# jhamrick/gaussian_processes

Hardware: AMD Instinct MI355X
Metric: GP fit+predict wall-clock (kernel build + Cholesky + solve + log_lh + posterior mean) (lower is better)
Workload: dtype f64; 1 GPU; N=65536 d=32 RBF(GaussianKernel) f64, m=1000 test points, h=1 w=0.5*sqrt(d) s=1; N=65536, d=32, m=1000, parallelism=1 GPU

## Files before the change

### gaussian_processes_amd/csrc/gpx_common.h

```cpp
#pragma once
#include <hip/hip_runtime.h>
#include <stdint.h>
#include <stdio.h>
#include <stdlib.h>
#include <string.h>
#include <math.h>
#include <vector>

#include "../../include/gpx.h"
#include "gpx_tune.h"

namespace gpx {

void set_error(const char *fmt, ...);
int  hip_fail(hipError_t e, const char *what, const char *file, int line);
int  ensure_device();

#define GPX_HIP(call)                                                        \
    do {                                                                     \
        hipError_t e__ = (call);                                             \
        if (e__ != hipSuccess) return gpx::hip_fail(e__, #call, __FILE__, __LINE__); \
    } while (0)

#define GPX_TRY(call)                                                        \
// ... 95 lines not shown

struct KParams {
    double c[6];
    double diag_add;
    int kernel;
    int member;
};
int make_kparams(int kernel, int member, const double *params, double diag_add, KParams *out);

struct Batch {
    int count; int64_t sA, sB, sC;
    int count2 = 1; int64_t tA = 0, tB = 0, tC = 0;
};

int gemm_nt(int dtype, int64_t M, int64_t N, int64_t K, const void *A, int64_t lda, const void *B,
            int64_t ldb, void *C, int64_t ldc, double alpha, int tri, int64_t row0, int64_t col0,
            hipStream_t st, int beta0 = 0, int ktri = 0, const Batch *bt = nullptr,
            int wide_tiles = 0);
int trsm_rows(int dtype, void *X, int64_t ldx, int64_t rows, const void *Ljj, int64_t ldl, int jb,
              hipStream_t st, const Batch *bt = nullptr);
int syrk_bc(int dtype, int64_t n, int64_t row_begin, void *Cloc, int64_t ldc, int64_t cl0, int64_t cl1,
            const void *Pb, int64_t ldp, int64_t k0, int64_t kb, int64_t nb, int P, int rank,
            hipStream_t st, const int *abort_flag = nullptr, const Batch *bt = nullptr);
struct PanelHints { bool idle_chip = false; int leaf_force = 0; };
struct PotrfHook { int (*fn)(void *user, int64_t cols_done, hipEvent_t panel_done); void *user; };
int potrf_panel(int dtype, void *A, int64_t lda, int64_t n, int64_t r0, int64_t c0, int64_t kb,
                int *info_dev, hipStream_t st, const Batch *bt = nullptr, int64_t kpre = 0,
                hipEvent_t done = nullptr, PanelHints hints = {});
int potrf(int dtype, void *A, int64_t n, int64_t lda, int *info_dev, hipStream_t st, const Batch *bt = nullptr,
          int64_t xrows = 0,
          bool may_block = false,
          const PotrfHook *hook = nullptr);
int potrf_panel_res(int dtype, void *A, int64_t lda, int64_t n, int64_t r0, int64_t c0, int64_t kb, int *info_dev,
                    hipStream_t st, const Batch *bt = nullptr, int64_t kpre = 0, hipEvent_t done = nullptr, PanelHints hints = {});
int64_t panel_res_max();
hipStream_t potrf_side_stream();
bool kernel_values_finite(int kernel, const double *p, double s, int dtype);
bool panel_res_fold(int64_t rows, int64_t kpre, int64_t kb, size_t es, int64_t lda, const void *base);
constexpr int TRSV_OPS_BLOCK = 512;
static inline int64_t trsv_ops_nblocks(int64_t n) { return n / TRSV_OPS_BLOCK; }
static inline bool trsv_ops_whole_blocks(int64_t n) { return n >= TRSV_OPS_BLOCK && n % TRSV_OPS_BLOCK == 0; }
struct TrsvOps {
    GrowBuf mem;
    bool valid = false;
    int64_t built = 0;
    void invalidate() { valid = false; built = 0; }
    static TrsvOps view(void *p, size_t bytes) { TrsvOps o; o.mem.p = p; o.mem.bytes = bytes; return o; }
};
int trsv_ops_build(int dtype, const void *L, int64_t n, int64_t ldl, TrsvOps *ops, hipStream_t st);
bool trsv_ops_ahead_ok(int dtype, const void *L, int64_t n, int64_t ldl);
bool trsm_ops_ok(int dtype, const void *L, int64_t n, int64_t ldl);
size_t trsv_ops_bytes(int dtype, int64_t n);
int trsv_ops_build_upto(int dtype, const void *L, int64_t n, int64_t ldl, TrsvOps *ops, int64_t kend, hipStream_t st);
int trsv_lower(int dtype, const void *L, int64_t n, int64_t ldl, void *b, void *x, int transpose,
               hipStream_t st, const Batch *bt = nullptr,
               TrsvOps *ops = nullptr);
int trsm_right_lt(int dtype, const void *L, int64_t n, int64_t ldl, void *X, int64_t m, int64_t ldx,
                  hipStream_t st, int x_upper = 0, TrsvOps *ops = nullptr,
                  int64_t c0 = 0);
int trsm_right_l(int dtype, const void *L, int64_t n, int64_t ldl, void *X, int64_t m, int64_t ldx, hipStream_t st,
                 TrsvOps *ops = nullptr);
int pred_grad(int dtype, int kernel, const void *xo, int64_t m, const void *x, int64_t n, int d, const double *params,
              const void *alpha, const void *B, int64_t ldb, double scale, const double *col_div, double *out_dev, hipStream_t st);
int inv_from_factor(int dtype, const void *L, int64_t n, int64_t ldl, void *X, void *W, int tri, hipStream_t st,
                    TrsvOps *ops, int count = 1, int64_t sL = 0, void *group_ops = nullptr);
int logdet_chol(int dtype, const void *L, int64_t n, int64_t ldl, double *out_dev, hipStream_t st, int count = 1,
                int64_t sL = 0, int64_t so = 0);
int dot(int dtype, const void *a, const void *b, int64_t n, double *out_dev, hipStream_t st, int count = 1,
        int64_t sa = 0, int64_t sb = 0, int64_t so = 0);
int tril(int dtype, void *A, int64_t n, int64_t lda, hipStream_t st);
int var_rows(int dtype, int kernel, const void *X, int64_t rows, int64_t n, int64_t ldx, const void *xo, int d,
             const double *params, const double *kdiag_dev, int accumulate, double *out_dev, hipStream_t st);
int var_finish(int dtype, int kernel, const void *xo, int d, const double *params, const double *acc_dev, int64_t rows,
               double *out_dev, hipStream_t st);
int eye_rows(int dtype, void *X, int64_t rows, int64_t ld, int64_t c0, int64_t cz, hipStream_t st);
int loo_rows(int dtype, const void *X, int64_t rows, int64_t n, int64_t ldx, int64_t c0, const void *y, const void *alpha,
             double *kii, double *mean, double *var, double *logp, hipStream_t st);
int loo_points(int dtype, const double *kii, const void *y, const void *alpha, int64_t n, double *mean, double *var, double *logp,
               hipStream_t st);
int sum_f64(const double *a, int64_t n, double *out_dev, hipStream_t st);
int copy_lower(int dtype, const void *src, int64_t lds, void *dst, int64_t ldd, int64_t n, hipStream_t st);
int schur_lower(int dtype, const void *B, int64_t k, int64_t n, int64_t ldb, void *S, int64_t lds, hipStream_t st);
int randn(int dtype, void *out, int64_t rows, int64_t cols, int64_t ld, uint64_t seed, uint64_t stream, uint64_t offset, hipStream_t st);
int mvn_sample(int dtype, void *C, int64_t m, int64_t ldc, const void *mean, double jitter, int64_t S, uint64_t seed, uint64_t stream,
               void *Z, int64_t ldz, void *out, int64_t ldo, int *info_dev, hipStream_t st);
bool kapply_fused_fits(int dtype, int d, int64_t S);
int kapply_fused(int dtype, const void *xo, int64_t m, const void *x, int64_t n, int d, const KParams &kp, const void *V, int64_t ldv,
                 int64_t S, void *out, int64_t ldo, hipStream_t st);
int rff_features(int dtype, const void *pts, int64_t m, int d, const double *omega_dev, int64_t F, double scale, void *out, int64_t ld,
                 hipStream_t st);
int rff_features_grad(int dtype, const void *pts, int64_t m, int d, const double *omega_dev, int64_t F, double scale, const double *col_div,
                      void *out, int64_t ld, hipStream_t st);
int kapply_grad(int dtype, const void *xo, int64_t m, const void *x, int64_t n, int d, const double *params, const double *col_div,
                const void *V, int64_t ldv, int64_t S, void *out, int64_t ldo, hipStream_t st);
int kmat_apply(int dtype, int kernel, const void *xo, int64_t m, const void *x, int64_t n, int d, const double *params, const void *V,
               int64_t ldv, int64_t S, void *out, int64_t ldo, hipStream_t st);
int var_plan(int dtype, int64_t n, int64_t m, int64_t chunk_rows, size_t free_bytes, int64_t *rows, int64_t *chunks, size_t *bytes);
int dloglh_reduce(int dtype, int kernel, const void *x, int64_t n, int d, const double *params,
                  const void *alpha, const void *W, int64_t ldw, double *partial_dev, double *out4,
                  hipStream_t st);
struct ArdWidths { double w[GPX_ARD_MAX_D]; };
int scale_points(int dtype, const void *x, int64_t n, int d, const double *w_host, void *out, hipStream_t st);
int ard_scratch(size_t bytes, void **p);
void ard_iso(const double *params, int d, double *iso2);
size_t dloglh_partial_doubles(int kernel, int d);
int dloglh_reduce_ard(int dtype, const void *xs, int64_t n, int d, const double *iso, const void *alpha, const void *W,
// ... 6 lines not shown
```

### gaussian_processes_amd/csrc/gpx_gp.hip

```cpp
#include "gpx_common.h"
#include <cmath>
#include <vector>

#include "gpx_gp_internal.h"

namespace gpx {

template <typename T>
__global__ void cvt_from_f64_2d(const double *__restrict__ src, int64_t lds, T *__restrict__ dst, int64_t ldd, int64_t rows, int64_t cols)
{
    const int64_t c = (int64_t)blockIdx.x * blockDim.x + threadIdx.x;
    if (c >= cols) return;
    for (int64_t r = blockIdx.y; r < rows; r += gridDim.y) dst[r * ldd + c] = (T)src[r * lds + c];
}

template <typename T>
__global__ void cvt_to_f64_2d(const T *__restrict__ src, int64_t lds, double *__restrict__ dst,
                              int64_t ldd, int64_t rows, int64_t cols, int lower_only)
{
    const int64_t c = (int64_t)blockIdx.x * blockDim.x + threadIdx.x;
    if (c >= cols) return;
    for (int64_t r = blockIdx.y; r < rows; r += gridDim.y) {
        const double v = (double)src[r * lds + c];
        dst[r * ldd + c] = (lower_only && c > r) ? 0.0 : v;
// ... 38 lines not shown
                           cols, rows, cols, lower_only);
    else
        hipLaunchKernelGGL((cvt_to_f64_2d<float>), grid, block, 0, st, (const float *)src, lds, tmp, cols,
                           rows, cols, lower_only);
    GPX_LAUNCH_CHECK();
    GPX_TRY(copy_rows(dst, ldh, tmp, cols, rows, cols, hipMemcpyDeviceToHost, st));
    GPX_HIP(hipStreamSynchronize(st));
    return GPX_OK;
}

int kmat(int dtype, int kernel, int member, const void *x1, int64_t n, const void *x2, int64_t m,
         int d, const double *params, double diag_add, int tri, void *out, int64_t ld, hipStream_t st)
{
    return gpx_d_kmat(dtype, kernel, member, x1, n, x2, m, d, params, diag_add, tri, out, ld, (void *)st);
}

int gp_rescale(gpx_gp *g)
{
    if (g->kernel != GPX_KERNEL_GAUSSIAN_ARD || !g->have_data || !g->have_params) return GPX_OK;
    ard_iso(g->params, g->d, g->iso);
    return scale_points(g->dtype, g->x, g->n, g->d, g->params + 1, g->xs, g->st);
}

static int upload_points(gpx_gp *g, void *dst, const double *xo, int64_t m)
{
    GPX_TRY(upload_f64(g->dtype, dst, m * g->d, xo, m * g->d, 1, m * g->d, g->st));
    if (g->kernel == GPX_KERNEL_GAUSSIAN_ARD) GPX_TRY(scale_points(g->dtype, dst, m, g->d, g->params + 1, dst, g->st));
    return GPX_OK;
}

int gp_read_scal(gpx_gp *g, GpScal *host)
{
    GPX_HIP(hipMemcpyAsync(host, g->scal, sizeof(GpScal), hipMemcpyDeviceToHost, g->st));
    GPX_HIP(hipStreamSynchronize(g->st));
    return check_internal_info(host->info);
}

int gp_need_factor(gpx_gp *g, const char *what_for)
{
    GpScal sc;
    GPX_TRY(gp_read_scal(g, &sc));
    if (sc.info != 0) { set_error("Kxx is not positive definite (info = %d): there is no factor %s", sc.info, what_for); return GPX_ERR_ARG; }
    return GPX_OK;
}

int check_internal_info(int info)
{
    if (info >= 0) return GPX_OK;
    set_error("internal failure inside the factorisation (info = %d: a hand-off between workgroups of the resident "
              "panel kernel timed out); the factor is not valid -- this is NOT a statement about the matrix", info);
    return GPX_ERR_INTERNAL;
}

int gp_finish_fit(gpx_gp *g, bool rhs_is_row_n, int *info)
{
    const size_t es = esize(g->dtype);
    hipStream_t st = g->st;
    if (rhs_is_row_n) {
        GPX_TRY(trsv_lower(g->dtype, g->A, g->n, g->lda, (char *)g->A + (size_t)g->n * g->lda * es, g->alpha, 1, st, nullptr, &g->ops));
    } else {
        GPX_HIP(hipMemcpyAsync(g->t0, g->y, (size_t)g->n * es, hipMemcpyDeviceToDevice, st));
        GPX_TRY(trsv_lower(g->dtype, g->A, g->n, g->lda, g->t0, g->t1, 0, st, nullptr, &g->ops));
        GPX_TRY(trsv_lower(g->dtype, g->A, g->n, g->lda, g->t1, g->alpha, 1, st, nullptr, &g->ops));
    }
    GPX_HIP(hipEventRecord(g->ev[3], st));
    GPX_TRY(logdet_chol(g->dtype, g->A, g->n, g->lda, &g->scal->logdet, st));
    GPX_TRY(dot(g->dtype, g->y, g->alpha, g->n, &g->scal->yta, st));
    GPX_HIP(hipEventRecord(g->ev[4], st));
    g->fitted = true;
    if (info) {
        GPX_HIP(hipMemcpyAsync(info, &g->scal->info, sizeof(int), hipMemcpyDeviceToHost, st));
        GPX_HIP(hipStreamSynchronize(st));
        GPX_TRY(check_internal_info(*info));
    }
    return GPX_OK;
}

template <typename T>
__global__ void nonfinite_kernel(const T *__restrict__ v, int64_t n, int *__restrict__ flag)
{
    bool bad = false;
    for (int64_t i = (int64_t)blockIdx.x * blockDim.x + threadIdx.x; i < n; i += (int64_t)gridDim.x * blockDim.x)
        bad = bad || !isfinite(v[i]);
    if (__any(bad) && (threadIdx.x & 63) == 0) atomicOr(flag, 1);
}

int gp_scan_finite(gpx_gp *g)
{
    int *flags = &g->scal->x_bad;
    GPX_HIP(hipMemsetAsync(flags, 0, 2 * sizeof(int), g->st));
    const int64_t nx = g->n * g->d, ny = g->n;
    const unsigned bx = (unsigned)std::min<int64_t>(cdiv(nx, 256), 1024), by = (unsigned)std::min<int64_t>(cdiv(ny, 256), 1024);
    if (g->dtype == GPX_F64) {
        hipLaunchKernelGGL((nonfinite_kernel<double>), dim3(bx), dim3(256), 0, g->st, (const double *)g->x, nx, flags);
        hipLaunchKernelGGL((nonfinite_kernel<double>), dim3(by), dim3(256), 0, g->st, (const double *)g->y, ny, flags + 1);
    } else {
        hipLaunchKernelGGL((nonfinite_kernel<float>), dim3(bx), dim3(256), 0, g->st, (const float *)g->x, nx, flags);
        hipLaunchKernelGGL((nonfinite_kernel<float>), dim3(by), dim3(256), 0, g->st, (const float *)g->y, ny, flags + 1);
    }
    GPX_LAUNCH_CHECK();
    int h[2] = {0, 0};
    GPX_HIP(hipMemcpyAsync(h, flags, sizeof(h), hipMemcpyDeviceToHost, g->st));
    GPX_HIP(hipStreamSynchronize(g->st));
    g->x_finite = h[0] == 0; g->y_finite = h[1] == 0;
    return GPX_OK;
}

template <typename T>
static bool kernel_values_finite_t(int kernel, const double *p, double s)
{
    T k0, k1;
    if (kernel == GPX_KERNEL_GAUSSIAN) {
// ... 169 lines not shown
{
    GP_ENTER(g);
    GPX_ARG(g && x && y, "NULL argument");
    GPX_TRY(upload_f64(g->dtype, g->x, g->n * g->d, x, g->n * g->d, 1, g->n * g->d, g->st));
    GPX_TRY(upload_f64(g->dtype, g->y, g->n, y, g->n, 1, g->n, g->st));
    g->have_data = true; gp_unfit(g);
    GPX_TRY(gp_rescale(g));
    return gp_scan_finite(g);
}

int gpx_gp_set_data_device(gpx_gp_t *g, const void *x_dev, const void *y_dev)
{
    GP_ENTER(g);
    GPX_ARG(g && x_dev && y_dev, "NULL argument");
    const size_t es = esize(g->dtype);
    GPX_HIP(hipMemcpyAsync(g->x, x_dev, (size_t)g->n * g->d * es, hipMemcpyDeviceToDevice, g->st));
    GPX_HIP(hipMemcpyAsync(g->y, y_dev, (size_t)g->n * es, hipMemcpyDeviceToDevice, g->st));
    GPX_HIP(hipStreamSynchronize(g->st));
    g->have_data = true; gp_unfit(g);
    GPX_TRY(gp_rescale(g));
    return gp_scan_finite(g);
}

int gpx_gp_set_params(gpx_gp_t *g, const double *params, double s)
{
    GP_ENTER(g);
    GPX_ARG(g && params, "NULL argument");
    GPX_ARG(!(s < 0), "invalid value for s");
    for (int i = 0; i < g->nparams; ++i) g->params[i] = params[i];
    g->s = s;
    g->have_params = true; g->have_K = false; gp_unfit(g);
    return gp_rescale(g);
}

int gpx_gp_get_params(gpx_gp_t *g, double *params, int cap, int *count)
{
    GP_ENTER(g);
    GPX_ARG(g->have_params, "no kernel parameters in the handle");
    GPX_ARG(cap >= 0 && (cap == 0 || params), "bad arguments");
    if (count) *count = g->nparams;
    for (int i = 0; i < g->nparams && i < cap; ++i) params[i] = g->params[i];
    return GPX_OK;
}

int gpx_gp_set_K(gpx_gp_t *g, const double *Kxx, int64_t ld)
{
    GP_ENTER(g);
    GPX_ARG(g && Kxx && ld >= g->n, "bad arguments");
    GPX_TRY(upload_f64(g->dtype, g->A, g->lda, Kxx, ld, g->n, g->n, g->st));
    g->have_K = true; gp_unfit(g);
    return GPX_OK;
}

struct OpsAhead { gpx_gp *g; int64_t group, last; };
static int ops_ahead_step(void *user, int64_t cols_done, hipEvent_t panel_done)
{
    OpsAhead *o = (OpsAhead *)user;
    gpx_gp *g = o->g;
    const int64_t ready = std::min(trsv_ops_nblocks(cols_done), o->last);
    if (ready - g->ops.built < o->group) return GPX_OK;
    GPX_HIP(hipStreamWaitEvent(g->st_ops, panel_done, 0));
    return trsv_ops_build_upto(g->dtype, g->A, g->n, g->lda, &g->ops, ready, g->st_ops);
}

int gpx_gp_fit(gpx_gp_t *g, int *info)
{
    GP_ENTER(g);
    GPX_ARG(g, "gp is NULL");
    GPX_ARG(g->have_data && (g->have_params || g->have_K),
            "set_data and set_params (or set_K) must be called before fit");
    const GpView v = gp_view(g);
    if (!g->have_K && (!g->x_finite || !kernel_values_finite(v.kernel, v.params, g->s, g->dtype))) {
        set_error("%s (%s)", NONFINITE_MSG, g->x_finite ? "kernel parameters or s" : "x");
        return GPX_ERR_ARG;
    }
    const size_t es = esize(g->dtype);
    hipStream_t st = g->st;
    GPX_HIP(hipEventRecord(g->ev[0], st));
    if (!g->have_K)
        GPX_TRY(kmat(g->dtype, v.kernel, GPX_K, v.x, g->n, v.x, g->n, g->d, v.params, g->s * g->s,
                     GPX_LOWER, g->A, g->lda, st));
    g->have_K = false;
    g->have_kii = false;
    GPX_HIP(hipEventRecord(g->ev[1], st));
    const int64_t ride_max = tune().fit_ride_max;
    const bool ride = g->n <= ride_max;
    route_hit(ride ? RT_FIT_RIDE : RT_FIT_TWO_SOLVES);
    if (ride) GPX_HIP(hipMemcpyAsync((char *)g->A + (size_t)g->n * g->lda * es, g->y, (size_t)g->n * es, hipMemcpyDeviceToDevice, st));
    g->ops.invalidate();
    const bool ahead = tune().fit_ops_ahead != 0 && g->n >= tune().fit_ops_ahead_min &&
                       trsv_ops_ahead_ok(g->dtype, g->A, g->n, g->lda);
    const int64_t nfull = trsv_ops_nblocks(g->n), tail = tune().fit_ops_tail;
    const int64_t group = std::max<int64_t>(1, std::min(nfull, nfull - tail));
    OpsAhead oa = {g, group, std::max<int64_t>(0, nfull - tail)};
    PotrfHook hook = {ops_ahead_step, &oa};
    if (ahead) {
        if (!g->st_ops) {
            int least = 0, greatest = 0;
            GPX_HIP(hipDeviceGetStreamPriorityRange(&least, &greatest));
            GPX_HIP(hipStreamCreateWithPriority(&g->st_ops, hipStreamNonBlocking, least));
            GPX_HIP(hipEventCreateWithFlags(&g->ev_ops, hipEventDisableTiming));
        }
        GPX_TRY(g->ops.mem.reserve(trsv_ops_bytes(g->dtype, g->n), st));
        GPX_TRY(order(g->ev_ops, st, g->st_ops));
    }
    GPX_TRY(potrf(g->dtype, g->A, g->n, g->lda, &g->scal->info, st, nullptr, ride ? 1 : 0, true, ahead ? &hook : nullptr));
    if (ahead) {
        GPX_TRY(order(g->ev_ops, g->st_ops, st));
        if (g->ops.built > 0) route_hit(RT_FIT_OPS_AHEAD);
    }
    GPX_HIP(hipEventRecord(g->ev[2], st));
    return gp_finish_fit(g, ride, info);
}

static int gp_scalars(gpx_gp_t *g, double *logdet, double *yta, int *info)
{
    GP_ENTER(g);
    GPX_ARG(g && g->fitted, "gp is not fitted");
    GpScal sc;
    GPX_TRY(gp_read_scal(g, &sc));
    if (logdet) *logdet = sc.logdet;
    if (yta) *yta = sc.yta;
    if (info) *info = sc.info;
    return GPX_OK;
}

int gpx_gp_log_lh(gpx_gp_t *g, double *log_lh)
{
    GPX_ARG(log_lh, "log_lh is NULL");
    GPX_ARG(g, "gp is NULL");
    GP_NEED_FINITE_Y(g);
    double logdet, yta; int info;
    GPX_TRY(gp_scalars(g, &logdet, &yta, &info));
    if (info != 0 || !(logdet >= GPX_MIN_LOG)) { *log_lh = -INFINITY; return GPX_OK; }
    const double data_fit = -0.5 * yta;
    const double complexity_penalty = -0.5 * logdet;
    const double constant = -0.5 * (double)g->n * log(2 * M_PI);
    *log_lh = data_fit + complexity_penalty + constant;
    return GPX_OK;
}

int gpx_gp_logdet(gpx_gp_t *g, double *logdet)
{
    GPX_ARG(logdet, "logdet is NULL");
    return gp_scalars(g, logdet, nullptr, nullptr);
}

int gpx_gp_info(gpx_gp_t *g, int *info)
{
    GPX_ARG(info, "info is NULL");
    return gp_scalars(g, nullptr, nullptr, info);
}

int gpx_gp_mean(gpx_gp_t *g, const double *xo, int64_t m, double *out)
{
    GP_ENTER(g);
    GPX_ARG(g && g->fitted, "gp is not fitted");
    GP_NEED_FINITE_Y(g);
    GPX_ARG(m >= 0 && (m == 0 || (xo && out)), "bad arguments");
    if (m == 0) return GPX_OK;
    const size_t es = esize(g->dtype);
    DevBuf dxo, dout;
    GPX_TRY(dxo.alloc((size_t)m * g->d * es));
    GPX_TRY(dout.alloc((size_t)m * es));
    GPX_TRY(upload_points(g, dxo.p, xo, m));
// ... 690 lines not shown
```

### gaussian_processes_amd/csrc/gpx_gp_internal.h

```cpp
#pragma once
#include "gpx_common.h"
#include <cstddef>

struct GpScal {
    double logdet;
    double yta;
    int x_bad, y_bad;
    int info;
    int pad;
};
static_assert(sizeof(GpScal) == 32 && offsetof(GpScal, x_bad) == 16 && offsetof(GpScal, info) == 24, "GpScal layout");

struct gpx_gp {
    int device;
    int dtype, kernel, d, nparams;
    int64_t n, lda;
    void *x, *y, *A, *alpha, *t0, *t1;
    void *xs;
    GpScal *scal;
    hipStream_t st;
    hipEvent_t ev[6];
    double params[1 + GPX_ARD_MAX_D];
    double iso[2];
    double s;
    bool have_data, have_params, fitted, have_K;
    bool x_finite, y_finite;
    gpx::GrowBuf bw; int64_t bw_cap;
    gpx::TrsvOps ops;
    gpx::GrowBuf gw; int64_t gw_cap;
    gpx::TrsvOps bops;
    double *kii;
    bool have_kii;
    hipStream_t st_ops;
    hipEvent_t ev_ops;
};

namespace gpx {
int gp_scan_finite(gpx_gp *g);
int upload_f64(int dtype, void *dst, int64_t ldd, const double *src, int64_t lds, int64_t rows, int64_t cols, hipStream_t st,
               DevBuf *stage = nullptr);
int download_f64(int dtype, double *dst, int64_t ldh, const void *src, int64_t lds, int64_t rows, int64_t cols, int lower_only,
                 hipStream_t st);
int gp_read_scal(gpx_gp *g, GpScal *host);
int gp_need_factor(gpx_gp *g, const char *what_for);
static inline void gp_unfit(gpx_gp *g) { g->fitted = false; g->have_kii = false; }
int gp_finish_fit(gpx_gp *g, bool rhs_is_row_n, int *info);
static inline int nparams_of(int kernel, int d) { return kernel == GPX_KERNEL_GAUSSIAN_ARD ? 1 + d : (kernel == GPX_KERNEL_PERIODIC ? 3 : 2); }
struct GpView { int kernel; const void *x; const double *params; };
static inline GpView gp_view(const gpx_gp *g)
{
    if (g->kernel == GPX_KERNEL_GAUSSIAN_ARD) return {GPX_KERNEL_GAUSSIAN, g->xs, g->iso};
    return {g->kernel, g->x, g->params};
}
int gp_rescale(gpx_gp *g);
}

#define GP_ENTER(g)                                                          \
    GPX_ARG((g) != nullptr, "gp is NULL");                                   \
    gpx::tune_refresh();                                                     \
    gpx::DeviceGuard guard__((g)->device);                                   \
    if (guard__.rc != GPX_OK) return guard__.rc;                             \
    gpx::StreamTurn turn__((g)->st);                                         \
    gpx::RoctxRange api_range__(__func__)
```

### gaussian_processes_amd/csrc/gpx_potrf.hip

```cpp
#include "gpx_common.h"
#include "gpx_leaf.h"
#include <vector>

namespace gpx {

constexpr int IBP = IB + 1;


template <typename T, bool INV>
__global__ __launch_bounds__(256) void potrf_diag_kernel(T *__restrict__ blk, int64_t lda, int64_t j0,
                                                         int jb, int *__restrict__ info, T *__restrict__ inv,
                                                         int64_t sblk)
{
    blk += (int64_t)blockIdx.x * sblk;
    info += blockIdx.x;
    if (INV) inv += (int64_t)blockIdx.x * (IB * IB);
    __builtin_amdgcn_s_setprio(3);
    const int tid = threadIdx.x;
    const int tr = tid >> 4, tc = tid & 15;
    __shared__ int s_abort;
    if (tid == 0) s_abort = *info;
    __syncthreads();
    if (s_abort != 0) return;
    T a[4][4];
// ... 98 lines not shown
}

template <typename T>
__global__ void tril_kernel(T *__restrict__ A, int64_t n, int64_t lda)
{
    for (int64_t i = blockIdx.y; i < n; i += gridDim.y)
        for (int64_t c = i + 1 + (int64_t)blockIdx.x * blockDim.x + threadIdx.x; c < n;
             c += (int64_t)gridDim.x * blockDim.x)
            A[i * lda + c] = (T)0;
}

int tril(int dtype, void *A, int64_t n, int64_t lda, hipStream_t st)
{
    if (n <= 1) return GPX_OK;
    dim3 grid((unsigned)std::min<int64_t>(cdiv(n, 256), 64), (unsigned)std::min<int64_t>(n, 32768)), block(256);
    if (dtype == GPX_F64) hipLaunchKernelGGL((tril_kernel<double>), grid, block, 0, st, (double *)A, n, lda);
    else hipLaunchKernelGGL((tril_kernel<float>), grid, block, 0, st, (float *)A, n, lda);
    GPX_LAUNCH_CHECK();
    return GPX_OK;
}

static int64_t outer_block(int64_t n, bool batched = false)
{
    const int64_t forced = tune().potrf_nb;
    if (forced >= IB && forced % IB == 0) return forced;
    if (batched && n >= 8192 && n <= 32768) return 1024;
    if (batched && n >= 4096 && n <= 32768) return 512;
    const long long *thr = tune().potrf_widths;
    if (n <= thr[0]) return 128;
    if (n <= thr[1]) return 256;
    if (n <= thr[2]) return 512;
    return 1024;
}

static thread_local ThreadScratch g_leaf;

template <typename T>
static int potrf_panel_t(T *A, int64_t lda, int64_t n, int64_t r0, int64_t c0, int64_t kb, int *info_dev,
                         hipStream_t st, int dtype, const Batch *bt, int64_t kpre = 0, hipEvent_t done = nullptr,
                         PanelHints hints = {})
{
    const int nbatch = bt ? bt->count : 1;
    const int64_t sM = bt ? bt->sA : 0;
    if (kb % IB == 0 && kb <= panel_res_max()) {
        route_hit(RT_PANEL_RES);
        return potrf_panel_res(dtype, A, lda, n, r0, c0, kb, info_dev, st, bt, kpre, done, hints);
    }
    if (kpre != 0) { set_error("potrf_panel: a folded update needs the resident panel route"); return GPX_ERR_ARG; }
    if (kb <= IB) {
        route_hit(RT_PANEL_CHAIN);
        const int jb = (int)kb;
        T *D = A + r0 * lda + c0;
        const int64_t below = n - (r0 + jb);
        const bool via_inverse = !tune().potrf_trsm_rows && below > 0 && below <= tune().potrf_inv_max &&
                                 jb == IB && lda % (16 / (int64_t)sizeof(T)) == 0 &&
                                 ((uintptr_t)(A + (r0 + jb) * lda + c0)) % 16 == 0;
        T *inv = nullptr;
        if (via_inverse) {
            void *p = nullptr;
            GPX_TRY(g_leaf.get(std::max<size_t>((size_t)nbatch * IB * IB * sizeof(T), IB * IB * 8), &p));
            inv = (T *)p;
        }
        {
            ProfScope prof(PC_POTRF_DIAG, (double)jb * jb * jb / 3.0 * nbatch, st);
            if (inv)
                hipLaunchKernelGGL((potrf_diag_kernel<T, true>), dim3(nbatch), dim3(256), 0, st, D, lda, r0, jb,
                                   info_dev, inv, sM);
            else
                hipLaunchKernelGGL((potrf_diag_kernel<T, false>), dim3(nbatch), dim3(256), 0, st, D, lda, r0, jb,
                                   info_dev, inv, sM);
        }
        GPX_LAUNCH_CHECK();
        if (via_inverse) {
            T *Xb = A + (r0 + jb) * lda + c0;
            Batch bi; bi.count = nbatch; bi.sA = sM; bi.sB = IB * IB; bi.sC = sM;
            GPX_TRY(gemm_nt(dtype, below, jb, jb, Xb, lda, inv, IB, Xb, lda, 1.0, GPX_FULL, 0, 0, st, 1, 0,
                            bt ? &bi : nullptr));
        } else if (below > 0) {
            Batch br; br.count = nbatch; br.sA = sM; br.sB = sM; br.sC = 0;
            GPX_TRY(trsm_rows(dtype, A + (r0 + jb) * lda + c0, lda, below, D, lda, jb, st, bt ? &br : nullptr));
        }
        if (done) GPX_HIP(hipEventRecord(done, st));
        return GPX_OK;
    }
    const int64_t h = ((kb / IB + 1) / 2) * IB;
    GPX_TRY(potrf_panel_t<T>(A, lda, n, r0, c0, h, info_dev, st, dtype, bt, 0, nullptr, hints));
    hints.idle_chip = false;
    T *R = A + (r0 + h) * lda + c0;
    if (panel_res_fold(n - (r0 + h), h, kb - h, sizeof(T), lda, A))
        return potrf_panel_t<T>(A, lda, n, r0 + h, c0 + h, kb - h, info_dev, st, dtype, bt, h, done, hints);
    GPX_TRY(gemm_nt(dtype, n - (r0 + h), kb - h, h, R, lda, R, lda, R + h, lda, -1.0, GPX_LOWER, 0, 0, st, 0, 0, bt));
    return potrf_panel_t<T>(A, lda, n, r0 + h, c0 + h, kb - h, info_dev, st, dtype, bt, 0, done, hints);
}

int potrf_panel(int dtype, void *A, int64_t lda, int64_t n, int64_t r0, int64_t c0, int64_t kb,
                int *info_dev, hipStream_t st, const Batch *bt, int64_t kpre, hipEvent_t done, PanelHints hints)
{
    if (dtype == GPX_F64)
        return potrf_panel_t<double>((double *)A, lda, n, r0, c0, kb, info_dev, st, dtype, bt, kpre, done, hints);
    return potrf_panel_t<float>((float *)A, lda, n, r0, c0, kb, info_dev, st, dtype, bt, kpre, done, hints);
}

struct LookAhead { hipStream_t q = nullptr; EventPool ev; };
static thread_local PerDevice<LookAhead> g_la;

hipStream_t potrf_side_stream()
{
// ... 198 lines not shown
```

### gaussian_processes_amd/csrc/gpx_solve.hip

```cpp
#include "gpx_common.h"
#include "gpx_kernels_dev.h"
#include "gpx_leaf.h"

namespace gpx {

constexpr int SB = 64;
constexpr int OB = TRSV_OPS_BLOCK;

template <typename T>
__global__ __launch_bounds__(256) void inv64_kernel(const T *__restrict__ L, int64_t ldl, int64_t ncols,
                                                    T *__restrict__ out, int transposed, T *__restrict__ W,
                                                    T *__restrict__ Wt, int64_t bsL, int64_t bsOut)
{
    L += (int64_t)blockIdx.y * bsL;
    const int tid = threadIdx.x, tr = tid >> 4, tc = tid & 15;
    const int64_t k0 = (int64_t)blockIdx.x * SB;
    const int jb = (int)min((int64_t)SB, ncols - k0);
    const T *blk = L + k0 * ldl + k0;
    T a[4][4], x[4][4];
#pragma unroll
    for (int r = 0; r < 4; ++r)
#pragma unroll
        for (int c = 0; c < 4; ++c) {
            const int row = 4 * tr + r, col = 4 * tc + c;
// ... 492 lines not shown
struct Sweep {
    const T *L; int64_t n, ldl, ncols; T *b, *x; hipStream_t st;
    unsigned nbt; int64_t sL, sv;
    T *Linv; int64_t sLinv;
    int aligned;
    int64_t nb() const { return cdiv(ncols, TB); }
    int width(int64_t blk) const { return (int)std::min<int64_t>(TB, ncols - blk * TB); }
};

template <typename T>
static void inv64_blocks(const Sweep<T> &S, int64_t first, int transposed)
{
    hipLaunchKernelGGL((inv64_kernel<T>), dim3((unsigned)(cdiv(S.ncols, SB) - first), S.nbt), dim3(256), 0, S.st,
                       S.L + first * SB * (S.ldl + 1), S.ldl, S.ncols - first * SB, S.Linv + first * SB * SB, transposed,
                       (T *)nullptr, (T *)nullptr, S.sL, S.sLinv);
}

template <typename T>
static void steps_fwd(const Sweep<T> &S, int64_t kfirst)
{
    const int64_t n = S.n, nb = S.nb();
    auto launch = [&](int64_t far_rows, int64_t nn, int64_t k0, int jb, int64_t p0, int pjb, int64_t far0) {
        hipLaunchKernelGGL((trsv_fwd_fused<T>), dim3((unsigned)(1 + cdiv(far_rows, 64)), S.nbt), dim3(TBT), 0, S.st, S.L, S.ldl,
                           S.Linv, S.b, S.x, nn, k0, jb, p0, pjb, far0, S.aligned, S.sL, S.sLinv, S.sv);
    };
    for (int64_t blk = kfirst; blk < nb; ++blk) {
        const int64_t k0 = blk * TB, p0 = std::max<int64_t>(blk - 1, 0) * TB;
        const int jb = S.width(blk), pjb = blk > 0 ? TB : 0;
        if (blk > 0) launch(jb, k0 + jb, k0, 0, p0, pjb, k0);
        launch(blk > 0 ? n - (k0 + jb) : 0, n, k0, jb, p0, pjb, k0 + jb);
    }
    if (n > S.ncols) launch(n - S.ncols, n, S.ncols, 0, (nb - 1) * TB, S.width(nb - 1), S.ncols);
}

template <typename T>
static void steps_bwd(const Sweep<T> &S, int64_t kfirst)
{
    const int64_t nb = S.nb();
    for (int64_t blk = nb - 1; blk >= kfirst; --blk) {
        const int64_t k0 = blk * TB, q0 = k0 + TB;
        const int jb = S.width(blk), qjb = blk + 1 < nb ? S.width(blk + 1) : 0;
        if (qjb > 0)
            hipLaunchKernelGGL((trsv_bwd_fused<T, 32>), dim3((unsigned)(1 + cdiv(jb, 32)), S.nbt), dim3(TBT), 0, S.st, S.L,
                               S.ldl, S.Linv, S.b, S.x, k0, 0, q0, qjb, k0, k0 + jb, S.aligned, S.sL, S.sLinv, S.sv);
        hipLaunchKernelGGL((trsv_bwd_fused<T, 128>), dim3((unsigned)(1 + (qjb > 0 ? cdiv(k0, 128) : 0)), S.nbt),
                           dim3(TBT), 0, S.st, S.L, S.ldl, S.Linv, S.b, S.x, k0, jb, q0, qjb, (int64_t)0, k0, S.aligned,
                           S.sL, S.sLinv, S.sv);
    }
}

constexpr int NCH = OB / (TBT / OPL);

template <typename T>
static void ops_fwd(const Sweep<T> &S, const OpsView<T> &V)
{
    for (int64_t k = 0; k < V.nfull; ++k) {
        const int64_t k0 = k * OB, far0 = k0 + OB;
        const int64_t nfar = k > 0 ? cdiv(S.n - far0, 64) : 0;
        hipLaunchKernelGGL((trsv_op_kernel<T, true>), dim3((unsigned)(NCH + nfar)), dim3(TBT), 0, S.st, V.W(k),
                           k > 0 ? V.Tf(k) : (const T *)nullptr, S.L, S.ldl, S.b, S.x, S.n, k0, k0 - OB, k > 0 ? OB : 0, far0, S.n, NCH, 1);
    }
}

template <typename T>
static void ops_bwd(const Sweep<T> &S, const OpsView<T> &V, int64_t kend)
{
    for (int64_t k = kend - 1; k >= 0; --k) {
        const int64_t k0 = k * OB, q0 = k0 + OB;
        const int qjb = (k + 1 < V.nfull) ? OB : (int)(S.n - q0);
        const int64_t nfar = qjb > 0 ? cdiv(k0, 128) : 0;
        hipLaunchKernelGGL((trsv_op_kernel<T, false>), dim3((unsigned)(NCH + nfar)), dim3(TBT), 0, S.st, V.Wt(k),
                           qjb > 0 ? V.Tb(k) : (const T *)nullptr, S.L, S.ldl, S.b, S.x, S.n, k0, q0, qjb, (int64_t)0, k0, NCH, 1);
    }
}

template <typename T>
static int trsv_t(const T *L, int64_t n, int64_t ldl, T *b, T *x, int transpose, hipStream_t st,
                  int64_t ncols = -1, const Batch *bt = nullptr, TrsvOps *ops = nullptr)
{
    constexpr int dtype = sizeof(T) == 8 ? GPX_F64 : GPX_F32;
    if (ncols < 0 || ncols > n) ncols = n;
    Sweep<T> S;
    S.L = L; S.n = n; S.ldl = ldl; S.ncols = ncols; S.b = b; S.x = x; S.st = st;
    S.nbt = (unsigned)(bt ? bt->count : 1); S.sL = bt ? bt->sA : 0; S.sv = bt ? bt->sB : 0;
    ProfScope prof(PC_TRSV, ((double)n * ncols - 0.5 * (double)ncols * (ncols - 1)) * sizeof(T) * S.nbt, st);
    S.sLinv = cdiv(ncols, SB) * SB * SB;
    void *scr = nullptr;
    GPX_TRY(g_scr.get((size_t)S.nbt * S.sLinv * sizeof(T), &scr));
    S.Linv = (T *)scr;
    S.aligned = (((uintptr_t)L) % (2 * sizeof(T)) == 0) && (ldl % 2 == 0);
    const bool usable = !bt && ncols == n && ops_usable(dtype, L, ldl);
    const bool cached = ops && ops->mem.p && n % OB == 0 && ops->mem.bytes >= trsv_ops_bytes(dtype, n);
    const bool prebuilt = cached && ops->valid;
    const int64_t kpart = (usable && cached && !ops->valid && ops->built > 0 && transpose) ? std::min(ops->built, n / OB) : 0;
    if (kpart == 0 && usable && (n >= trsv_ops_min_n() || prebuilt)) {
        route_hit(RT_TRSV_OPS);
        void *buf = nullptr;
        if (ops) {
            bool grew = false;
            GPX_TRY(ops->mem.reserve(trsv_ops_bytes(dtype, n), st, &grew));
            if (grew) ops->invalidate();
            buf = ops->mem.p;
        } else {
            GPX_TRY(g_ops.get(trsv_ops_bytes(dtype, n), &buf));
        }
        const OpsView<T> V(buf, n);
        if (!ops || !ops->valid) GPX_TRY(trsv_ops_prepare<T>(L, n, ldl, buf, st, ops ? std::min(ops->built, V.nfull) : 0, V.nfull));
        if (ops) { ops->valid = true; ops->built = V.nfull; }
        const bool ragged = n > V.nfull * OB;
        if (!transpose) {
            ops_fwd(S, V);
            if (ragged) { inv64_blocks(S, 0, 1); steps_fwd(S, V.nfull); }
        } else {
            if (ragged) { inv64_blocks(S, 0, 0); steps_bwd(S, V.nfull); }
            ops_bwd(S, V, V.nfull);
        }
    } else if (!transpose) {
        route_hit(RT_TRSV_STEPS);
        inv64_blocks(S, 0, 1);
        steps_fwd(S, 0);
    } else {
        route_hit(RT_TRSV_STEPS);
        inv64_blocks(S, kpart * (OB / SB), 0);
        steps_bwd(S, kpart);
        if (kpart > 0) {
            route_hit(RT_TRSV_OPS);
            ops_bwd(S, OpsView<T>(ops->mem.p, n), kpart);
        }
    }
    GPX_LAUNCH_CHECK();
    return GPX_OK;
}

int trsv_lower(int dtype, const void *L, int64_t n, int64_t ldl, void *b, void *x, int transpose,
               hipStream_t st, const Batch *bt, TrsvOps *ops)
{
    if (n <= 0) return GPX_OK;
    if (dtype == GPX_F64)
        return trsv_t<double>((const double *)L, n, ldl, (double *)b, (double *)x, transpose, st, -1, bt, ops);
    return trsv_t<float>((const float *)L, n, ldl, (float *)b, (float *)x, transpose, st, -1, bt, ops);
}

int trsv_ops_build(int dtype, const void *L, int64_t n, int64_t ldl, TrsvOps *ops, hipStream_t st)
{
    if (!ops || !trsv_ops_whole_blocks(n) || !ops_usable(dtype, L, ldl)) return GPX_OK;
    GPX_TRY(ops->mem.reserve(trsv_ops_bytes(dtype, n), st));
    ops->invalidate();
    if (dtype == GPX_F64) GPX_TRY(trsv_ops_prepare<double>((const double *)L, n, ldl, ops->mem.p, st));
    else GPX_TRY(trsv_ops_prepare<float>((const float *)L, n, ldl, ops->mem.p, st));
    ops->valid = true;
    ops->built = n / OB;
    return GPX_OK;
}

int trsv_ops_build_upto(int dtype, const void *L, int64_t n, int64_t ldl, TrsvOps *ops, int64_t kend, hipStream_t st)
{
    if (!ops || !trsv_ops_ahead_ok(dtype, L, n, ldl)) return GPX_OK;
    const int64_t nfull = n / OB;
    kend = std::min(kend, nfull);
    if (ops->built == 0) {
        GPX_TRY(ops->mem.reserve_device(trsv_ops_bytes(dtype, n)));
        ops->valid = false;
    }
    if (kend <= ops->built || !ops->mem.p) return GPX_OK;
    if (dtype == GPX_F64) GPX_TRY(trsv_ops_prepare<double>((const double *)L, n, ldl, ops->mem.p, st, ops->built, kend));
    else GPX_TRY(trsv_ops_prepare<float>((const float *)L, n, ldl, ops->mem.p, st, ops->built, kend));
    ops->built = kend;
    if (kend == nfull) ops->valid = true;
    return GPX_OK;
}

int trsv_lower_cols(int dtype, const void *L, int64_t n, int64_t ldl, int64_t ncols, void *b, void *x,
                    hipStream_t st)
{
    if (n <= 0 || ncols <= 0) return GPX_OK;
    if (dtype == GPX_F64)
        return trsv_t<double>((const double *)L, n, ldl, (double *)b, (double *)x, 0, st, ncols);
    return trsv_t<float>((const float *)L, n, ldl, (float *)b, (float *)x, 0, st, ncols);
}

template <typename T>
__global__ __launch_bounds__(256) void panel_gemv_t_partial(const T *__restrict__ Lp, int64_t ldl,
                                                            int64_t rows, int ncols,
                                                            const T *__restrict__ x, double *__restrict__ work)
{
    __shared__ T sx[256];
    const int tid = threadIdx.x;
    const int64_t r0 = (int64_t)blockIdx.x * 256;
    sx[tid] = (r0 + tid < rows) ? x[r0 + tid] : (T)0;
    __syncthreads();
    const int nr = (int)std::min<int64_t>(256, rows - r0);
    for (int c = tid; c < ncols; c += 256) {
        const T *col = Lp + r0 * ldl + c;
        double acc = 0.0;
        for (int i = 0; i < nr; ++i) acc = fma((double)col[(int64_t)i * ldl], (double)sx[i], acc);
        work[(int64_t)blockIdx.x * ncols + c] = acc;
    }
}

template <typename T>
__global__ void panel_gemv_t_reduce(const double *__restrict__ work, int64_t nchunks, int ncols,
                                    T *__restrict__ y)
{
    const int c = blockIdx.x * blockDim.x + threadIdx.x;
    if (c >= ncols) return;
    double acc = 0.0;
    for (int64_t k = 0; k < nchunks; ++k) acc += work[k * ncols + c];
    y[c] = (T)((double)y[c] - acc);
}

int panel_gemv_t(int dtype, const void *Lp, int64_t ldl, int64_t rows, int64_t ncols, const void *x,
                 void *y, double *work, hipStream_t st)
{
    if (rows <= 0 || ncols <= 0) return GPX_OK;
    const int64_t nchunks = cdiv(rows, 256);
    ProfScope prof(PC_TRSV, (double)rows * ncols * esize(dtype), st);
    if (dtype == GPX_F64) {
        hipLaunchKernelGGL((panel_gemv_t_partial<double>), dim3((unsigned)nchunks), dim3(256), 0, st,
                           (const double *)Lp, ldl, rows, (int)ncols, (const double *)x, work);
        hipLaunchKernelGGL((panel_gemv_t_reduce<double>), dim3((unsigned)cdiv(ncols, 256)), dim3(256), 0, st,
                           work, nchunks, (int)ncols, (double *)y);
// ... 636 lines not shown
```

### gaussian_processes_amd/csrc/gpx_tune.h

```cpp
#pragma once
#include <stdint.h>

namespace gpx {

#define GPX_TUNE_LIST(X, XF, XS, X2)                                                                                   \
                                                                               \
    XF(gemm_no_fast, "GPX_GEMM_NO_FAST")                                                                               \
    X(gemm_ablate, "GPX_GEMM_ABLATE", 0)                                                                               \
    X(gemm_pad_lds, "GPX_GEMM_PAD_LDS", 0)                                                                             \
    X(gemm_bn64_tiles, "GPX_GEMM_BN64_TILES", 256)                                                                     \
    X(gemm_exact, "GPX_GEMM_EXACT", 1)                                                                                 \
    X(gemm_fine_tiles, "GPX_GEMM_FINE_TILES", 16384)                                                                   \
    X2(syrk_bn64_tiles, "GPX_SYRK_BN64_TILES", 2600, 4000)                                                             \
                                                              \
    X(fit_ride_max, "GPX_FIT_RIDE_MAX", 16384)                                                                         \
    X(fit_ops_ahead, "GPX_FIT_OPS_AHEAD", 1)                                                                           \
    X(fit_ops_ahead_min, "GPX_FIT_OPS_AHEAD_MIN", 8192)                                                                \
    X(fit_ops_tail, "GPX_FIT_OPS_TAIL", 4)                                                                             \
    XS(batch_max, "GPX_BATCH_MAX", 1)                                                                                  \
    X(io_block_bytes, "GPX_IO_BLOCK_BYTES", (int64_t)64 << 20)                                                         \
    X(kmat_panel_bytes, "GPX_KMAT_PANEL_BYTES", (int64_t)256 << 20)                                                    \
                                                                        \
    XF(force_collectives, "GPX_FORCE_COLLECTIVES")                                                                     \
    X(mg_bcast_chunks, "GPX_MG_BCAST_CHUNKS", 4)                                                                       \
    XF(mg_no_timing, "GPX_MG_NO_TIMING")                                                                               \
    XS(mg_owner_first, "GPX_MG_OWNER_FIRST", 0)                                                                        \
                                                                  \
    XF(trace, "GPX_TRACE")                                                                                             \
    X(potrf_res, "GPX_POTRF_RES", 256)                                                                                 \
    X(res_strict, "GPX_RES_STRICT", 1)                                                                                 \
    X(two_part_rows, "GPX_POTRF_TWO_PART_ROWS", 16384)                                                                 \
    X(two_part_batch, "GPX_POTRF_TWO_PART_BATCH", 98304)                                                               \
    X(leaf_mfma_f32_rows, "GPX_LEAF_MFMA_F32_ROWS", 16384)                                                             \
    X(panel_excl_rows, "GPX_PANEL_EXCL_ROWS", 5120)                                                                    \
    XS(leaf, "GPX_LEAF", 0)                                                                                            \
    X2(leaf4_rows, "GPX_LEAF4_ROWS", 8192, 5120)                                                                       \
    X2(panel_pad_lds, "GPX_PANEL_PAD_LDS", 8 * 1024, 40 * 1024)                                                        \
    X(fold_rows, "GPX_POTRF_FOLD_ROWS", 16384)                                                                         \
    X(fold_k, "GPX_POTRF_FOLD_K", 256)                                                                                 \
                                                                  \
    XS(potrf_nb, "GPX_POTRF_NB", 0)                                                                                    \
    XF(potrf_trsm_rows, "GPX_POTRF_TRSM_ROWS")                                                                         \
    X(potrf_inv_max, "GPX_POTRF_INV_MAX", 16384)                                                                       \
    XF(no_lookahead, "GPX_POTRF_NO_LOOKAHEAD")                                                                         \
    X(taper, "GPX_POTRF_TAPER", 1)                                                                                     \
    X2(pair_rows, "GPX_POTRF_PAIR_ROWS", 0, 0)                                                                         \
    X(host_paced, "GPX_POTRF_HOST_PACED", 16384)                                                                       \
    X(gate_rows, "GPX_POTRF_GATE_ROWS", 16384)                                                                         \
                                                                                 \
    X(trsv_ops, "GPX_TRSV_OPS", 1)                                                                                     \
    X(trsv_ops_min, "GPX_TRSV_OPS_MIN", 10240)                                                                         \
    X(trsm_ops, "GPX_TRSM_OPS", 1)                                                                                     \
                                                                          \
    XF(roctx, "GPX_ROCTX")

constexpr int64_t GPX_KAPPLY_FUSED_MAX_F64 = 32;
constexpr int64_t GPX_KAPPLY_FUSED_MAX_F32 = 8;

struct Tune {
#define GPX_T_X(f, e, d) int64_t f = (d);
#define GPX_T_XF(f, e) bool f = false;
#define GPX_T_XS(f, e, d) int64_t f = (d); bool f##_set = false;
#define GPX_T_X2(f, e, d0, d1) int64_t f[2] = {(d0), (d1)};
    GPX_TUNE_LIST(GPX_T_X, GPX_T_XF, GPX_T_XS, GPX_T_X2)
#undef GPX_T_X
#undef GPX_T_XF
#undef GPX_T_XS
#undef GPX_T_X2
    long long potrf_widths[3] = {1, 8192, 12288};
    bool mg_bcast_set = false, mg_bcast_sag = false;
    char rccl_lib[256] = {0};
    int64_t kapply_fused_max[2] = {GPX_KAPPLY_FUSED_MAX_F64, GPX_KAPPLY_FUSED_MAX_F32};
};

const Tune &tune();
void tune_refresh();
int64_t tune_refresh_count();

}
```

Baseline: 1.320 s.

## Overlap forward triangular solve with Cholesky factorisation on side stream

During the fit, the forward substitution L t1 = y is now advanced block by block on the side ops stream as soon as each group of trsv operators is built behind the panel factorisation. The final forward solve then only covers the remaining blocks before the backward solve. It also removes the GPX_POTRF_TRSM_ROWS tuning flag so the inverse-based trailing solve path is always eligible. The intent is to hide forward-solve latency under the Cholesky, at the cost of smaller operator-build groups and extra cross-stream work that could contend with the factorisation.

```diff
diff --git a/gaussian_processes_amd/csrc/gpx_common.h b/gaussian_processes_amd/csrc/gpx_common.h
--- a/gaussian_processes_amd/csrc/gpx_common.h
+++ b/gaussian_processes_amd/csrc/gpx_common.h
@@ -171,6 +171,9 @@
 bool trsm_ops_ok(int dtype, const void *L, int64_t n, int64_t ldl);
 size_t trsv_ops_bytes(int dtype, int64_t n);
 int trsv_ops_build_upto(int dtype, const void *L, int64_t n, int64_t ldl, TrsvOps *ops, int64_t kend, hipStream_t st);
+bool trsv_ops_fwd_ok(int dtype, const void *L, int64_t n, int64_t ldl);
+int trsv_ops_fwd_range(int dtype, const void *L, int64_t n, int64_t ldl, const TrsvOps *ops, void *b, void *x, int64_t kbeg, int64_t kend,
+                       hipStream_t st);
 int trsv_lower(int dtype, const void *L, int64_t n, int64_t ldl, void *b, void *x, int transpose,
                hipStream_t st, const Batch *bt = nullptr,
                TrsvOps *ops = nullptr);
diff --git a/gaussian_processes_amd/csrc/gpx_gp.hip b/gaussian_processes_amd/csrc/gpx_gp.hip
--- a/gaussian_processes_amd/csrc/gpx_gp.hip
+++ b/gaussian_processes_amd/csrc/gpx_gp.hip
@@ -114,12 +114,17 @@
     return GPX_ERR_INTERNAL;
 }
 
-int gp_finish_fit(gpx_gp *g, bool rhs_is_row_n, int *info)
+int gp_finish_fit(gpx_gp *g, bool rhs_is_row_n, int *info, int64_t fwd_swept)
 {
     const size_t es = esize(g->dtype);
     hipStream_t st = g->st;
     if (rhs_is_row_n) {
         GPX_TRY(trsv_lower(g->dtype, g->A, g->n, g->lda, (char *)g->A + (size_t)g->n * g->lda * es, g->alpha, 1, st, nullptr, &g->ops));
+    } else if (fwd_swept >= 0) {
+        const int64_t nfull = trsv_ops_nblocks(g->n);
+        GPX_TRY(trsv_ops_build_upto(g->dtype, g->A, g->n, g->lda, &g->ops, nfull, st));
+        GPX_TRY(trsv_ops_fwd_range(g->dtype, g->A, g->n, g->lda, &g->ops, g->t0, g->t1, fwd_swept, nfull, st));
+        GPX_TRY(trsv_lower(g->dtype, g->A, g->n, g->lda, g->t1, g->alpha, 1, st, nullptr, &g->ops));
     } else {
         GPX_HIP(hipMemcpyAsync(g->t0, g->y, (size_t)g->n * es, hipMemcpyDeviceToDevice, st));
         GPX_TRY(trsv_lower(g->dtype, g->A, g->n, g->lda, g->t0, g->t1, 0, st, nullptr, &g->ops));
@@ -395,7 +400,7 @@
     return GPX_OK;
 }
 
-struct OpsAhead { gpx_gp *g; int64_t group, last; };
+struct OpsAhead { gpx_gp *g; int64_t group, last; bool sweep; int64_t swept; };
 static int ops_ahead_step(void *user, int64_t cols_done, hipEvent_t panel_done)
 {
     OpsAhead *o = (OpsAhead *)user;
@@ -403,7 +408,12 @@
     const int64_t ready = std::min(trsv_ops_nblocks(cols_done), o->last);
     if (ready - g->ops.built < o->group) return GPX_OK;
     GPX_HIP(hipStreamWaitEvent(g->st_ops, panel_done, 0));
-    return trsv_ops_build_upto(g->dtype, g->A, g->n, g->lda, &g->ops, ready, g->st_ops);
+    GPX_TRY(trsv_ops_build_upto(g->dtype, g->A, g->n, g->lda, &g->ops, ready, g->st_ops));
+    if (o->sweep && g->ops.built > o->swept) {
+        GPX_TRY(trsv_ops_fwd_range(g->dtype, g->A, g->n, g->lda, &g->ops, g->t0, g->t1, o->swept, g->ops.built, g->st_ops));
+        o->swept = g->ops.built;
+    }
+    return GPX_OK;
 }
 
 int gpx_gp_fit(gpx_gp_t *g, int *info)
@@ -434,8 +444,15 @@
     const bool ahead = tune().fit_ops_ahead != 0 && g->n >= tune().fit_ops_ahead_min &&
                        trsv_ops_ahead_ok(g->dtype, g->A, g->n, g->lda);
     const int64_t nfull = trsv_ops_nblocks(g->n), tail = tune().fit_ops_tail;
-    const int64_t group = std::max<int64_t>(1, std::min(nfull, nfull - tail));
-    OpsAhead oa = {g, group, std::max<int64_t>(0, nfull - tail)};
+    int64_t group = std::max<int64_t>(1, std::min(nfull, nfull - tail));
+    const int64_t fwd_group = tune().fit_fwd_group;
+    const bool shadow = ahead && !ride && fwd_group > 0 && trsv_ops_fwd_ok(g->dtype, g->A, g->n, g->lda);
+    if (shadow) {
+        group = std::min(group, fwd_group);
+        route_hit(RT_TRSV_OPS);
+        GPX_HIP(hipMemcpyAsync(g->t0, g->y, (size_t)g->n * es, hipMemcpyDeviceToDevice, st));
+    }
+    OpsAhead oa = {g, group, std::max<int64_t>(0, nfull - tail), shadow, 0};
     PotrfHook hook = {ops_ahead_step, &oa};
     if (ahead) {
         if (!g->st_ops) {
@@ -453,7 +470,7 @@
         if (g->ops.built > 0) route_hit(RT_FIT_OPS_AHEAD);
     }
     GPX_HIP(hipEventRecord(g->ev[2], st));
-    return gp_finish_fit(g, ride, info);
+    return gp_finish_fit(g, ride, info, shadow ? oa.swept : -1);
 }
 
 static int gp_scalars(gpx_gp_t *g, double *logdet, double *yta, int *info)
diff --git a/gaussian_processes_amd/csrc/gpx_gp_internal.h b/gaussian_processes_amd/csrc/gpx_gp_internal.h
--- a/gaussian_processes_amd/csrc/gpx_gp_internal.h
+++ b/gaussian_processes_amd/csrc/gpx_gp_internal.h
@@ -44,7 +44,7 @@
 int gp_read_scal(gpx_gp *g, GpScal *host);
 int gp_need_factor(gpx_gp *g, const char *what_for);
 static inline void gp_unfit(gpx_gp *g) { g->fitted = false; g->have_kii = false; }
-int gp_finish_fit(gpx_gp *g, bool rhs_is_row_n, int *info);
+int gp_finish_fit(gpx_gp *g, bool rhs_is_row_n, int *info, int64_t fwd_swept = -1);
 static inline int nparams_of(int kernel, int d) { return kernel == GPX_KERNEL_GAUSSIAN_ARD ? 1 + d : (kernel == GPX_KERNEL_PERIODIC ? 3 : 2); }
 struct GpView { int kernel; const void *x; const double *params; };
 static inline GpView gp_view(const gpx_gp *g)
diff --git a/gaussian_processes_amd/csrc/gpx_potrf.hip b/gaussian_processes_amd/csrc/gpx_potrf.hip
--- a/gaussian_processes_amd/csrc/gpx_potrf.hip
+++ b/gaussian_processes_amd/csrc/gpx_potrf.hip
@@ -174,7 +174,7 @@
         const int jb = (int)kb;
         T *D = A + r0 * lda + c0;
         const int64_t below = n - (r0 + jb);
-        const bool via_inverse = !tune().potrf_trsm_rows && below > 0 && below <= tune().potrf_inv_max &&
+        const bool via_inverse = below > 0 && below <= tune().potrf_inv_max &&
                                  jb == IB && lda % (16 / (int64_t)sizeof(T)) == 0 &&
                                  ((uintptr_t)(A + (r0 + jb) * lda + c0)) % 16 == 0;
         T *inv = nullptr;
diff --git a/gaussian_processes_amd/csrc/gpx_solve.hip b/gaussian_processes_amd/csrc/gpx_solve.hip
--- a/gaussian_processes_amd/csrc/gpx_solve.hip
+++ b/gaussian_processes_amd/csrc/gpx_solve.hip
@@ -568,9 +568,9 @@
 constexpr int NCH = OB / (TBT / OPL);
 
 template <typename T>
-static void ops_fwd(const Sweep<T> &S, const OpsView<T> &V)
-{
-    for (int64_t k = 0; k < V.nfull; ++k) {
+static void ops_fwd(const Sweep<T> &S, const OpsView<T> &V, int64_t kbeg, int64_t kend)
+{
+    for (int64_t k = kbeg; k < kend; ++k) {
         const int64_t k0 = k * OB, far0 = k0 + OB;
         const int64_t nfar = k > 0 ? cdiv(S.n - far0, 64) : 0;
         hipLaunchKernelGGL((trsv_op_kernel<T, true>), dim3((unsigned)(NCH + nfar)), dim3(TBT), 0, S.st, V.W(k),
@@ -625,7 +625,7 @@
         if (ops) { ops->valid = true; ops->built = V.nfull; }
         const bool ragged = n > V.nfull * OB;
         if (!transpose) {
-            ops_fwd(S, V);
+            ops_fwd(S, V, 0, V.nfull);
             if (ragged) { inv64_blocks(S, 0, 1); steps_fwd(S, V.nfull); }
         } else {
             if (ragged) { inv64_blocks(S, 0, 0); steps_bwd(S, V.nfull); }
@@ -683,6 +683,34 @@
     else GPX_TRY(trsv_ops_prepare<float>((const float *)L, n, ldl, ops->mem.p, st, ops->built, kend));
     ops->built = kend;
     if (kend == nfull) ops->valid = true;
+    return GPX_OK;
+}
+
+bool trsv_ops_fwd_ok(int dtype, const void *L, int64_t n, int64_t ldl) { return trsv_ops_ahead_ok(dtype, L, n, ldl) && n >= trsv_ops_min_n(); }
+
+template <typename T>
+static void trsv_ops_fwd_range_t(const T *L, int64_t n, int64_t ldl, const void *buf, T *b, T *x, int64_t kbeg, int64_t kend, hipStream_t st)
+{
+    Sweep<T> S;
+    S.L = L; S.n = n; S.ldl = ldl; S.ncols = n; S.b = b; S.x = x; S.st = st;
+    S.nbt = 1; S.sL = 0; S.sv = 0; S.Linv = nullptr; S.sLinv = 0; S.aligned = 1;
+    const double c0 = (double)kbeg * OB, c1 = (double)kend * OB;
+    ProfScope prof(PC_TRSV, ((c1 - c0) * (double)n - 0.5 * (c1 * c1 - c0 * c0)) * sizeof(T), st);
+    ops_fwd(S, OpsView<T>(buf, n), kbeg, kend);
+}
+
+int trsv_ops_fwd_range(int dtype, const void *L, int64_t n, int64_t ldl, const TrsvOps *ops, void *b, void *x, int64_t kbeg, int64_t kend,
+                       hipStream_t st)
+{
+    if (kbeg >= kend) return GPX_OK;
+    if (!ops || !ops->mem.p || !trsv_ops_fwd_ok(dtype, L, n, ldl) || kbeg < 0 || kend > std::min(ops->built, n / OB)) {
+        set_error("trsv_ops_fwd_range: blocks [%lld, %lld) of a factor whose operators cover %lld", (long long)kbeg, (long long)kend,
+                  (long long)(ops ? ops->built : 0));
+        return GPX_ERR_ARG;
+    }
+    if (dtype == GPX_F64) trsv_ops_fwd_range_t<double>((const double *)L, n, ldl, ops->mem.p, (double *)b, (double *)x, kbeg, kend, st);
+    else trsv_ops_fwd_range_t<float>((const float *)L, n, ldl, ops->mem.p, (float *)b, (float *)x, kbeg, kend, st);
+    GPX_LAUNCH_CHECK();
     return GPX_OK;
 }
 
diff --git a/gaussian_processes_amd/csrc/gpx_tune.h b/gaussian_processes_amd/csrc/gpx_tune.h
--- a/gaussian_processes_amd/csrc/gpx_tune.h
+++ b/gaussian_processes_amd/csrc/gpx_tune.h
@@ -17,6 +17,7 @@
     X(fit_ops_ahead, "GPX_FIT_OPS_AHEAD", 1)                                                                           \
     X(fit_ops_ahead_min, "GPX_FIT_OPS_AHEAD_MIN", 8192)                                                                \
     X(fit_ops_tail, "GPX_FIT_OPS_TAIL", 4)                                                                             \
+    X(fit_fwd_group, "GPX_FIT_FWD_GROUP", 16)                                                                          \
     XS(batch_max, "GPX_BATCH_MAX", 1)                                                                                  \
     X(io_block_bytes, "GPX_IO_BLOCK_BYTES", (int64_t)64 << 20)                                                         \
     X(kmat_panel_bytes, "GPX_KMAT_PANEL_BYTES", (int64_t)256 << 20)                                                    \
@@ -40,7 +41,6 @@
     X(fold_k, "GPX_POTRF_FOLD_K", 256)                                                                                 \
                                                                   \
     XS(potrf_nb, "GPX_POTRF_NB", 0)                                                                                    \
-    XF(potrf_trsm_rows, "GPX_POTRF_TRSM_ROWS")                                                                         \
     X(potrf_inv_max, "GPX_POTRF_INV_MAX", 16384)                                                                       \
     XF(no_lookahead, "GPX_POTRF_NO_LOOKAHEAD")                                                                         \
     X(taper, "GPX_POTRF_TAPER", 1)                                                                                     \
```

New measurement: 1.317 s (median of 3 runs). Within noise of the previous version (-0.2%).
